# peterWon/LVI-ExC

Hardware: AMD Instinct MI355X
Metric: M residual+Jacobian evals/s per GN iter (higher is better)
Workload: dtype f64; 1 GPU; config4-full-LVI: 1000000 surfel + 200000 IMU samples (gyro+accel blocks) + 49992 ORB reprojection blocks, 25023 knots @ dt=0.02; step = residuals + analytic Jacobians + Huber + J^T J/J^T r assembly (no linear solve); n_tangent=155259, bandwidth=179, n_border=52, tracks=orb, parallelism=sequence-per-gpu x1, allreduce_transport=none (one sequence)

## Files before the change

lvi-exc_amd/csrc/lvx_api.hip:

```cpp
#include <algorithm>
#include <cmath>
#include <cstring>
#include <numeric>
#include <cstdlib>

#include "lvx_ctx.h"

namespace lvx {

#define LVX_SYNC_EVENT_FLAGS(c) hipEventDisableTiming
const SwitchName* switch_table(int* count) {
  static const SwitchName tab[] = {
    {"FORCE_LEGACY", &Switches::force_legacy, false}, {"SERIAL", &Switches::serial, false}, {"NO_GRAPH", &Switches::no_graph, false}, {"DETERMINISTIC", &Switches::deterministic, true},
    {"CLEAR_ALL", &Switches::clear_all, false}, {"SOLVER_SEQ", &Switches::solver_seq, false}, {"SOLVER_TIMING", &Switches::solver_timing, false},
    {"CHUNK_R", &Switches::chunk_r, true}, {"CHUNK_R_IMU", &Switches::chunk_r_imu, true}, {"CHUNK_R_REP", &Switches::chunk_r_rep, true}, {"CHUNK_ROWS", &Switches::chunk_rows, true}, {"REP_ROWS", &Switches::rep_rows, true}, {"REP_FUSED", &Switches::rep_fused, true}, {"SOLVER_ND", &Switches::solver_nd, false},
    {"DA_SYNC", &Switches::da_sync, false},
    {"TEST_BAD_PIVOT", &Switches::test_bad_pivot, false},
    {"TEST_COMPACT_ONE", &Switches::test_compact_one, false},
    {"TEST_LM_SCHUR_ONE", &Switches::test_lm_schur_one, false},
  };
  *count = (int)(sizeof(tab) / sizeof(tab[0]));
  return tab;
}
static void read_env_switches(lvx_ctx* c) {
  int n; const SwitchName* t = switch_table(&n);
  for (int i = 0; i < n; ++i) {
    const std::string name = std::string("LVX_") + t[i].name;
    if (const char* e = std::getenv(name.c_str())) c->sw.*(t[i].field) = (*e == 0) ? 1 : atoi(e);
  }
}

__global__ void k_checksum(const unsigned long long* p, size_t n, unsigned long long* out) {
  unsigned long long acc = 0;
  for (size_t i = (size_t)blockIdx.x * blockDim.x + threadIdx.x; i < n; i += (size_t)gridDim.x * blockDim.x) {
    unsigned long long b = p[i];
    if (b == 0x8000000000000000ull) b = 0;
    acc += b * (2ull * i + 1ull);
  }
  for (int o = 32; o > 0; o >>= 1) acc += __shfl_xor(acc, o);
  if ((threadIdx.x & 63) == 0) atomicAdd(out, acc);
}
__global__ void k_export_tail(const double* cost, const int* err, double* out) { out[0] = cost[0]; out[1] = (double)err[0]; }

}

using namespace lvx;

extern "C" {
// ... 428 lines not shown
```

lvi-exc_amd/csrc/lvx_ctx.h:

```cpp
#pragma once
#include <hip/hip_runtime.h>
#include <stdint.h>

#include <array>
#include <string>
#include <functional>
#include <vector>

#include "../../include/lvx.h"
#include "lvx_resid.h"

#define LVX_NREP 64
#define LVX_DEAD (-2147483647 - 1)
#define LVX_LM_BASE 0x40000000
#define LVX_ERR_FALLBACK 16

namespace lvx {

struct XbTab { int32_t* keys[LVX_NUM_FAM]; double* vals[LVX_NUM_FAM]; };
struct DevCommon {
  const double* state;
  int N, L;
  double t0, dt;
  uint32_t locks;
  uint32_t what;
  double imu_mto, sensor_mto;
  CamIntr cam;
  const int* ord;
  int nb, bw, nbd;
  int nbd_solve;
  int nrep;
  int hub_lo, hub_hi;
  const void* hubs;
  const So3Pre* pre;
  double* Hb;
  double* gb;
  double* Bd;
  double* C;
  double* gc;
  double* lmH; const int* lm_p0; int lm_wl, lm_ls;
  double* cost;
  int* err;
  int* fb_list; int fb_cap;
  double* residuals;
  int32_t* jcols;
  union {
    double* jvals;
    const XbTab* xb;
  };
};

struct DevBuf {
  void* p = nullptr;
  size_t bytes = 0;
};

struct Switches {
  int force_legacy = 0, serial = 0, no_graph = 0, deterministic = 0, clear_all = 0, solver_seq = 0, solver_timing = 0, chunk_r = 0, chunk_r_imu = 0, chunk_r_rep = 0, chunk_rows = 0, rep_rows = 0, da_sync = 0, rep_fused = 0, solver_nd = 0, test_bad_pivot = 0, test_compact_one = 0, test_lm_schur_one = 0;
};
struct SwitchName { const char* name; int Switches::*field; bool relayout; };
const SwitchName* switch_table(int* count);

struct Family {
  int n = 0;
  std::vector<double> t, a3, b3;
  std::vector<int32_t> id0, id1;
  double huber = 0, weight = 1;
  DevBuf d_t, d_a3, d_b3, d_id0, d_id1, d_perm;
};

}

struct lvx_ctx {
  int device = 0;
  hipStream_t stream = nullptr;
  hipStream_t own_stream = nullptr;
  hipStream_t fam_stream[4] = {nullptr, nullptr, nullptr, nullptr};
  hipEvent_t ev_fork = nullptr, ev_join[4] = {nullptr, nullptr, nullptr, nullptr}, ev_jac = nullptr;
  hipEvent_t ev_fb[2] = {nullptr, nullptr};
  std::string last_error;
  bool have_spline = false;
  double t0 = 0, dt = 1;
  int N = 0, L = 0;
  uint32_t locks = LVX_LOCK_LIDAR_TAU | LVX_LOCK_CAM_TAU;
  double imu_mto = 0.01, sensor_mto = 0.001;
  lvx::CamIntr cam{};
  lvx::Family imu, surf, rep, cs;
  lvx::Family lp; double lp_t_start = 0;
  lvx::DevBuf d_pairs_lp, d_lp_part, d_lp_out; double* h_lp = nullptr;
  bool has_prior = false;
  double prior_t = 0, prior_q[4] = {1, 0, 0, 0}, prior_w = 1;
// ... 134 lines not shown
```

lvi-exc_amd/csrc/lvx_eval.hip:

```cpp
#include <algorithm>
#include <cmath>
#include <cstring>
#include <functional>
#include <numeric>
#include <cstdlib>

#include <thread>
#include "lvx_ctx.h"

namespace lvx {

#define LVX_PW 4
struct Keys { int k0, k1, lm; };
LVX_HD bool same(const Keys& a, const Keys& b) { return a.k0 == b.k0 && a.k1 == b.k1 && a.lm == b.lm; }

struct Cal { ImuCal imu; SensorCal lidar, cam; const double* rho; };
__device__ __forceinline__ Cal load_cal(const DevCommon& cm) {
  const double* s = cm.state + 7 * (size_t)cm.N;
  Cal c;
  c.imu.tau = s[7]; c.imu.roll = s[8]; c.imu.pitch = s[9]; c.imu.ba = load_v3(s + 10); c.imu.bg = load_v3(s + 13);
  c.lidar.q = load_q(s + 16); c.lidar.p = load_v3(s + 20); c.lidar.tau = s[23];
  c.cam.q = load_q(s + 24); c.cam.p = load_v3(s + 28); c.cam.tau = s[31];
  c.rho = s + 32;
  return c;
// ... 1310 lines not shown
}

struct ImuG { enum { NR = 3, NCJ = GYRO_NC, NK = 12, NG = 3, KPK = 3, LVO = 3, GL = 32, GOFF = 5, NKL = 12, NCL = 16, NT = 1, NTP = 1, LDP = 18, PR = 96 }; };
struct ImuA { enum { NR = 3, NCJ = ACC_NC, NK = 24, NG = 5, KPK = 6, LVO = 0, GL = 16, GOFF = 0, NKL = 24, NCL = 30, NT = 2, NTP = 3, LDP = 34, PR = 48 }; };
#define IMU_NGA 8
struct ImuAccLds { double* band; double* bd; double* gg; double* gk; double* gG; int lv; };
template <class PG> __device__ __forceinline__ int imu_cls(int lc) {
  return lc < PG::NKL ? 6 * (lc / PG::KPK) + PG::LVO + lc % PG::KPK : (lc < PG::NKL + PG::NG ? -1 - (PG::GOFF + lc - PG::NKL) : (lc == PG::NKL + PG::NG ? -100 : -200));
}
template <class PG> __device__ __forceinline__ void imu_build_rtab(int* rtab, int lane, const double* sm, const ImuAccLds& A) {
  int t = 0;
#pragma unroll
  for (int ci = 0; ci < PG::NT; ++ci)
#pragma unroll
    for (int cj = ci; cj < PG::NT; ++cj, ++t)
#pragma unroll
      for (int v = 0; v < 4; ++v) {
        const int row = ci * 16 + (lane >> 4) + 4 * v, col = cj * 16 + (lane & 15);
        int ent = -1;
        if (!(ci == cj && col < row)) {
          const int ra = imu_cls<PG>(row), cb = imu_cls<PG>(col);
          if (ra >= 0) {
            if (cb >= 0) { const int d = cb - ra; if (d >= 0 && d < ACC_BW) ent = ((int)(A.band - sm) + ra * ACC_BW + d) | (2 << 16) | (cb << 18); }
            else if (cb > -100) ent = ((int)(A.bd - sm) + (-1 - cb) * A.lv + ra) | (1 << 16) | (ra << 18);
            else if (cb == -100) ent = ((int)(A.gk - sm) + ra) | (1 << 16) | (ra << 18);
          } else if (ra > -100) {
            if (cb > -100 && cb < 0) ent = (int)(A.gg - sm) + (-1 - ra) * IMU_NGA + (-1 - cb);
            else if (cb == -100) ent = (int)(A.gG - sm) + (-1 - ra);
          }
        }
        rtab[t * 4 + v] = ent;
      }
}
template <class PG> __device__ __forceinline__ void imu_assemble(double* sm, double* P, const int* rtab, bool valid, int key, int k_lo, int acc_lv, const double* r, const double (*J)[PG::NCJ], int lane, int dummy) {
  constexpr int NR = PG::NR, NT = PG::NT, LDP = PG::LDP, PR = PG::PR, GL = PG::GL;
  const unsigned long long vm = __ballot(valid);
  for (int g0 = 0; g0 < 64; g0 += GL) {
    const unsigned long long pmask = ((1ull << GL) - 1ull) << g0;
    unsigned long long rem = vm & pmask;
    if (!rem) continue;
    if (lane >= g0 && lane < g0 + GL) {
      const int li = lane - g0;
#pragma unroll
      for (int a = 0; a < NR; ++a) {
        double2* prow2 = (double2*)(P + (li * NR + a) * LDP);
        auto col = [&](int c) { return c < PG::NK + PG::NG ? (valid ? J[a][c] : 0.0) : (c == PG::NK + PG::NG ? (valid ? r[a] : 0.0) : 0.0); };
#pragma unroll
        for (int c2 = 0; c2 < 8 * NT; ++c2) prow2[c2] = make_double2(col(2 * c2), col(2 * c2 + 1));
      }
    }
    __builtin_amdgcn_fence(__ATOMIC_RELEASE, "wavefront");
    __builtin_amdgcn_wave_barrier();
    __builtin_amdgcn_fence(__ATOMIC_ACQUIRE, "wavefront");
    while (rem) {
      const int l0 = __ffsll((long long)rem) - 1;
      const int kw = __builtin_amdgcn_readfirstlane(__shfl(key, l0));
      const unsigned long long wm = __ballot(valid && key == kw) & pmask;
      rem &= ~wm;
      const int lhi = 63 - __clzll((long long)wm);
      const int wb = (kw - k_lo) * 6;
      const int r_lo = (l0 - g0) * NR, r_hi = (lhi - g0 + 1) * NR;
      const unsigned long long wsh = wm >> g0;
      const bool contig = __popcll(wm) == lhi - l0 + 1;
      d4 D[PG::NTP];
#pragma unroll
      for (int t = 0; t < PG::NTP; ++t) D[t] = d4{0.0, 0.0, 0.0, 0.0};
      const int nks = (r_hi - r_lo + 3) >> 2;
      auto trip = [&](int ks, auto UC) {
        constexpr int U = decltype(UC)::value;
        double f[U][NT];
#pragma unroll
        for (int q = 0; q < U; ++q) {
          const int rr = r_lo + 4 * (ks + q) + (lane >> 4);
          bool mine = rr < r_hi;
          if (!contig) mine = mine && ((wsh >> (rr / NR)) & 1ull);
          const double* src = P + min(rr, PR - 1) * LDP + (lane & 15);
#pragma unroll
          for (int c = 0; c < NT; ++c) { const double x = src[c * 16]; f[q][c] = mine ? x : 0.0; }
        }
#pragma unroll
        for (int q = 0; q < U; ++q) {
          int t = 0;
#pragma unroll
          for (int ci = 0; ci < NT; ++ci)
#pragma unroll
            for (int cj = ci; cj < NT; ++cj, ++t) D[t] = __builtin_amdgcn_mfma_f64_16x16x4f64(f[q][ci], f[q][cj], D[t], 0, 0, 0);
        }
      };
      int ks = 0;
      for (; ks + 6 <= nks; ks += 6) trip(ks, std::integral_constant<int, 6>{});
      for (; ks < nks; ks += 2) trip(ks, std::integral_constant<int, 2>{});
      const int wbB = wb * ACC_BW;
#pragma unroll
      for (int t = 0; t < PG::NTP; ++t)
#pragma unroll
        for (int v = 0; v < 4; ++v) {
          const int te = rtab[t * 4 + v];
          const bool ok = te >= 0 && wb + (te >> 18) < acc_lv;
          const int m = (te >> 16) & 3;
          const int idx = ok ? (te & 0xffff) + (m == 2 ? wbB : (m == 1 ? wb : 0)) : dummy + lane;
          atomicAdd(&sm[idx], ok ? D[t][v] : 0.0);
        }
    }
    __builtin_amdgcn_fence(__ATOMIC_RELEASE, "wavefront");
    __builtin_amdgcn_wave_barrier();
  }
}
struct ImuFused { int n; const double* t; const double* gyro; const double* acc; const int* perm; double w_gyro, w_acc; };
#define IMU_CR 32
#define IMU_LV ((IMU_CR + 5) * 6)
struct ImuOwn { const int* wg_c0; const int* own_k; int nch, span; };
#define LVX_LDS_BARRIER() asm volatile("s_waitcnt lgkmcnt(0)\n\ts_barrier" ::: "memory")
static size_t imu_fused_lds_bytes(int span) {
  const int pan = std::max((int)ImuG::PR * (int)ImuG::LDP, (int)ImuA::PR * (int)ImuA::LDP);
  return (size_t)(IMU_LV * ACC_BW + IMU_NGA * IMU_LV + IMU_NGA * IMU_NGA + IMU_LV + IMU_NGA + 64 + 4 * pan) * 8 + (size_t)span * sizeof(So3Pre) + (size_t)(7 * span + IMU_NGA) * 4 + 64;
}
__global__ void k_imu_rtab(int* out) {
  const int lane = threadIdx.x;
  const double* sm = (const double*)out;
  ImuAccLds A;
  A.band = (double*)sm; A.bd = A.band + IMU_LV * ACC_BW; A.gg = A.bd + IMU_NGA * IMU_LV; A.gk = A.gg + IMU_NGA * IMU_NGA; A.gG = A.gk + IMU_LV; A.lv = IMU_LV;
  int rtg[ImuG::NTP * 4], rta[ImuA::NTP * 4];
  imu_build_rtab<ImuG>(rtg, lane, sm, A);
  imu_build_rtab<ImuA>(rta, lane, sm, A);
  for (int i = 0; i < ImuG::NTP * 4; ++i) out[i * 64 + lane] = rtg[i];
  for (int i = 0; i < ImuA::NTP * 4; ++i) out[(ImuG::NTP * 4 + i) * 64 + lane] = rta[i];
}
template <bool EXP = false>
__global__ __launch_bounds__(256, 1) void k_imu_own(ImuFused fam, DevCommon cm, const int* __restrict__ chunk_off, ImuOwn ow, long long row0_g, long long row0_a, int det, const int* __restrict__ rtab_g) {
  constexpr int PAN = (ImuG::PR * ImuG::LDP > ImuA::PR * ImuA::LDP) ? ImuG::PR * ImuG::LDP : ImuA::PR * ImuA::LDP;
  constexpr int ACC_LV = IMU_LV, CR = IMU_CR, HB = ACC_BW / 2;
  extern __shared__ __attribute__((aligned(16))) double smo[];
  double* sm = smo;
  ImuAccLds A;
  A.band = sm; A.bd = A.band + ACC_LV * ACC_BW; A.gg = A.bd + IMU_NGA * ACC_LV; A.gk = A.gg + IMU_NGA * IMU_NGA; A.gG = A.gk + ACC_LV; A.lv = ACC_LV;
  double* panels = A.gG + IMU_NGA + 64;
  So3Pre* pre_all = (So3Pre*)(panels + 4 * PAN);
  int* kpos_all = (int*)(pre_all + ow.span);
  int* kown_all = kpos_all + 6 * ow.span;
  int* gpos = kown_all + ow.span;
  const int tid = threadIdx.x, lane = tid & 63, wv = tid >> 6;
  const int wg = blockIdx.x;
  const int c0 = ow.wg_c0[wg], c1 = ow.wg_c0[wg + 1];
  if (c0 >= c1) return;
  const int nwv = det ? 1 : 4;
  const bool want_ne = (cm.what & LVX_EVAL_NORMAL_EQ) != 0;
  constexpr int NACC = ACC_LV * ACC_BW + IMU_NGA * ACC_LV + IMU_NGA * IMU_NGA + ACC_LV + IMU_NGA;
  for (int e = tid; e < NACC; e += 256) sm[e] = 0.0;
  int* urng = gpos + IMU_NGA;
  if (tid < IMU_NGA) gpos[tid] = cm.ord[6 * cm.N + tid];
  if (tid == 0) { urng[0] = 1 << 30; urng[1] = -1; }
  const int k_base = chunk_off[ow.nch + 1 + c0] - 1;
  for (int e = tid; e < 6 * ow.span; e += 256) { const int kn = k_base + e / 6; kpos_all[e] = (kn >= 0 && kn < cm.N) ? cm.ord[6 * kn + e % 6] : LVX_DEAD; }
  for (int e = tid; e < ow.span; e += 256) {
    const int kn = k_base + e;
    kown_all[e] = (ow.own_k && kn >= 0 && kn < cm.N) ? ow.own_k[kn] : -1;
    if (kn >= 0 && kn + 1 < cm.N) pre_all[e] = cm.pre[kn];
    else { pre_all[e].Om = mk(0, 0, 0); pre_all[e].on = 0.0; pre_all[e].Jri = m3_identity(); pre_all[e].c3 = 1.0 / 12.0; pre_all[e].ok = 1; }
  }
  const SplineRef sp{cm.t0, cm.dt, cm.N, cm.state, cm.state + 3 * (size_t)cm.N};
  const Cal cal = load_cal(cm);
  if (fabs(cal.imu.tau) >= cm.dt && tid == 0) atomicOr(cm.err, LVX_ERR_FALLBACK);
  double* P = panels + wv * PAN;
  const int rep = wg % cm.nrep;
  int rtg[ImuG::NTP * 4], rta[ImuA::NTP * 4];
#pragma unroll
  for (int i = 0; i < ImuG::NTP * 4; ++i) rtg[i] = rtab_g[i * 64 + lane];
#pragma unroll
  for (int i = 0; i < ImuA::NTP * 4; ++i) rta[i] = rtab_g[(ImuG::NTP * 4 + i) * 64 + lane];
  double mycost = 0.0;
  const int ld = cm.bw + 1;
#ifdef LVX_KTIME_IMU
  long long kt_[12] = {0, 0, 0, 0, 0, 0, 0, 0, 0, 0, 0, 0}; long long kt0_ = __builtin_amdgcn_s_memtime(); const long long kts_ = kt0_;
#define IKT(i) { const long long n_ = __builtin_amdgcn_s_memtime(); kt_[i] += n_ - kt0_; kt0_ = n_; }
#else
#define IKT(i)
#endif
  for (int c = c0; c < c1; ++c) {
    const int m0 = chunk_off[c], m1 = chunk_off[c + 1];
    const int k_lo = chunk_off[ow.nch + 1 + c] - 1;
    const int woff = k_lo - k_base;
    const So3Pre* pre_tab = pre_all + woff;
    const int* kpos = kpos_all + 6 * woff;
    if (c == c0) __syncthreads(); else LVX_LDS_BARRIER();
    IKT(0)
    for (int base = wv < nwv ? m0 + wv * 64 : m1; base < m1; base += nwv * 64) {
      const int si = base + lane;
      const bool in = si < m1;
      int key = -1;
      bool valid = false;
      So3Eval e;
      KnotRef k;
      if (in) {
        int status = RES_OK;
        if (!knot_lookup(sp.t0, sp.dt, sp.n, fam.t[si], fam.t[si] + cal.imu.tau, &k)) status = RES_RANGE;
        else {
          key = k.i0;
          const So3Pre* pre = (k.i0 >= k_lo && k.i0 + 2 < k_lo + CR + 4) ? pre_tab + (k.i0 - k_lo) : nullptr;
          if (!pre) status = RES_OUTSIDE;
          else {
            quat cq[4]; load_so3_cp(sp, k.i0, cq);
            const int bad = so3_eval_pre<true, true>(cq, pre, k.u, sp.dt, &e);
            if (bad) status = (bad & 1) ? RES_NONUNIT : RES_OUTSIDE;
          }
        }
        valid = status == RES_OK;
        if (valid && (key < k_lo || key - k_lo > CR + 1)) { valid = false; fallback_row(cm, LVX_FAM_GYRO, si); }
        else if (!valid && status == RES_OUTSIDE) fallback_row(cm, LVX_FAM_GYRO, si);
        else if (!valid) atomicOr(cm.err, status);
      }
      IKT(1)
      {
        double r[3], J[3][GYRO_NC];
        if (valid) {
          const v3 wm = load_v3(fam.gyro + 3 * (size_t)si);
          const v3 pred = e.w_body + cal.imu.bg;
          const double w = fam.w_gyro;
          r[0] = w * (wm.x - pred.x); r[1] = w * (wm.y - pred.y); r[2] = w * (wm.z - pred.z);
#pragma unroll
          for (int kk = 0; kk < 4; ++kk)
#pragma unroll
            for (int a = 0; a < 3; ++a)
#pragma unroll
              for (int b = 0; b < 3; ++b) J[a][3 * kk + b] = -w * e.dw[kk].a[3 * a + b];
#pragma unroll
          for (int a = 0; a < 3; ++a)
#pragma unroll
            for (int b = 0; b < 3; ++b) J[a][12 + b] = (a == b) ? -w : 0.0;
          mycost += 0.5 * (r[0] * r[0] + r[1] * r[1] + r[2] * r[2]);
          if (cm.residuals) { const long long orow = row0_g + (long long)fam.perm[si] * 3; cm.residuals[orow] = r[0]; cm.residuals[orow + 1] = r[1]; cm.residuals[orow + 2] = r[2]; }
          if constexpr (EXP) put_record<3, GYRO_NC>(cm, LVX_FAM_GYRO, fam.perm[si], key, -1, -1, [&](int a, int c) { return J[a][c]; });
        }
        if constexpr (EXP) { if (in && !valid) { put_skipped(cm, LVX_FAM_GYRO, fam.perm[si]); put_skipped(cm, LVX_FAM_ACCEL, fam.perm[si]); } }
        if (want_ne) imu_assemble<ImuG>(sm, P, rtg, valid, key, k_lo, ACC_LV, r, J, lane, NACC);
        IKT(2)
      }
      {
        double r[3], J[3][ACC_NC];
        if (valid) {
          R3Basis b; r3_basis(k.u, sp.dt, &b);
          v3 acc = mk(0, 0, 0);
#pragma unroll
          for (int j = 0; j < 4; ++j) acc = acc + b.Ba[j] * load_v3(sp.r3 + 3 * (k.i0 + j));
          const v3 am = load_v3(fam.acc + 3 * (size_t)si);
          const double w = fam.w_acc;
          const double G = -9.79;
          const double cr = cos(cal.imu.roll), sr = sin(cal.imu.roll), cp = cos(cal.imu.pitch), sp_ = sin(cal.imu.pitch);
          const v3 g = mk(-sp_ * cr * G, sr * G, -cr * cp * G);
          const v3 y = acc + g;
          const v3 yb = qrot_inv(e.q, y);
          const v3 pred = yb + cal.imu.ba;
          r[0] = w * (am.x - pred.x); r[1] = w * (am.y - pred.y); r[2] = w * (am.z - pred.z);
          const m3 Rt = transpose(rotmat(e.q));
          const m3 S = skew(yb);
#pragma unroll
          for (int kk = 0; kk < 4; ++kk) {
            const m3 Mx = S * e.dxi[kk];
#pragma unroll
            for (int a = 0; a < 3; ++a)
#pragma unroll
              for (int bb = 0; bb < 3; ++bb) { J[a][6 * kk + bb] = -w * b.Ba[kk] * Rt.a[3 * a + bb]; J[a][6 * kk + 3 + bb] = -w * Mx.a[3 * a + bb]; }
          }
          const v3 dg_dr = Rt * mk(sp_ * sr * G, cr * G, sr * cp * G);
          const v3 dg_dp = Rt * mk(-cp * cr * G, 0.0, cr * sp_ * G);
#pragma unroll
          for (int a = 0; a < 3; ++a) {
            J[a][24] = -w * comp(dg_dr, a); J[a][25] = -w * comp(dg_dp, a);
#pragma unroll
            for (int bb = 0; bb < 3; ++bb) J[a][26 + bb] = (a == bb) ? -w : 0.0;
          }
          mycost += 0.5 * (r[0] * r[0] + r[1] * r[1] + r[2] * r[2]);
          if (cm.residuals) { const long long orow = row0_a + (long long)fam.perm[si] * 3; cm.residuals[orow] = r[0]; cm.residuals[orow + 1] = r[1]; cm.residuals[orow + 2] = r[2]; }
          if constexpr (EXP) put_record<3, ACC_NC>(cm, LVX_FAM_ACCEL, fam.perm[si], key, -1, -1, [&](int a, int c) { return J[a][c]; });
        }
        if (want_ne) imu_assemble<ImuA>(sm, P, rta, valid, key, k_lo, ACC_LV, r, J, lane, NACC);
        IKT(3)
      }
    }
    if (!want_ne) continue;
    int bt = tid; asm volatile("" : "+v"(bt));
    const bool more = c + 1 < c1;
    const int nfl = more ? min(ACC_LV, max(0, 6 * (chunk_off[ow.nch + 1 + c + 1] - 1 - k_lo))) : ACC_LV;
    const int* kown = kown_all + woff;
    const bool un_ = bt < nfl && kpos[bt] != LVX_DEAD && kown[bt / 6] != wg;
    { const unsigned long long ub = __ballot(un_);
      if (ub && lane == 0) { atomicMin(&urng[0], wv * 64 + __ffsll((long long)ub) - 1); atomicMax(&urng[1], wv * 64 + 63 - __clzll((long long)ub)); } }
    const int any_unowned = __syncthreads_or(un_);
    IKT(4)
    if (any_unowned) {
      const int r0 = urng[0], r1 = urng[1] + 1;
      for (int e = r0 * ACC_BW + bt; e < r1 * ACC_BW; e += 256) {
        const int la = e / ACC_BW, lb = la + e % ACC_BW;
        const int pa = kpos[la], o = kown[la / 6];
        if (o == wg || pa == LVX_DEAD || lb >= ACC_LV) continue;
        const double v = A.band[e];
        if (v == 0.0) continue;
        if (o >= 0) { atomicOr(cm.err, LVX_ERR_FALLBACK); continue; }
        const int pb = kpos[lb];
        if (pb != LVX_DEAD) add_H(cm, pa, pb, v, rep);
      }
      for (int gi = 0; gi < IMU_NGA; ++gi)
        for (int la = r0 + bt; la < r1; la += 256) {
          const int pg = gpos[gi], pa = kpos[la], o = kown[la / 6];
          if (pg == LVX_DEAD || pa == LVX_DEAD || (o == wg && pg < 0)) continue;
          const double v = A.bd[gi * ACC_LV + la];
          if (v == 0.0) continue;
          if (o >= 0) atomicOr(cm.err, LVX_ERR_FALLBACK); else add_H(cm, pg, pa, v, rep);
        }
      if (bt < nfl && kpos[bt] != LVX_DEAD && kown[bt / 6] != wg) {
        const double v = A.gk[bt];
        if (v != 0.0) { if (kown[bt / 6] >= 0) atomicOr(cm.err, LVX_ERR_FALLBACK); else add_g(cm, kpos[bt], v, rep); }
      }
      LVX_LDS_BARRIER();
      if (tid == 0) { urng[0] = 1 << 30; urng[1] = -1; }
    }
    IKT(6)
    {
      constexpr int NQB = (ACC_LV * HB + 255) / 256, NQD = (IMU_NGA * ACC_LV + 255) / 256;
      double2* band2 = (double2*)A.band;
      double2 vb[NQB]; int pb_[NQB], ob_[NQB];
#pragma unroll
      for (int q = 0; q < NQB; ++q) {
        const int e2 = bt + 256 * q;
        const bool inr = e2 < ACC_LV * HB;
        const int la = inr ? e2 / HB : 0;
        vb[q] = inr ? band2[e2] : make_double2(0.0, 0.0);
        pb_[q] = kpos[la]; ob_[q] = kown[la / 6];
        if (inr && more) band2[e2] = make_double2(0.0, 0.0);
      }
      double vd[NQD], vg = 0.0; int pd_[NQD], od_[NQD], pg_ = LVX_DEAD, og_ = -1;
#pragma unroll
      for (int q = 0; q < NQD; ++q) {
        const int e = bt + 256 * q;
        const bool inr = e < IMU_NGA * ACC_LV;
        const int la = inr ? e % ACC_LV : 0;
        vd[q] = inr ? A.bd[e] : 0.0;
        pd_[q] = kpos[la]; od_[q] = kown[la / 6];
        if (inr && more) A.bd[e] = 0.0;
      }
      if (bt < ACC_LV) { vg = A.gk[bt]; pg_ = kpos[bt]; og_ = kown[bt / 6]; if (more) A.gk[bt] = 0.0; }
      int gp_[NQD];
#pragma unroll
      for (int q = 0; q < NQD; ++q) { const int e = bt + 256 * q; gp_[q] = gpos[e < IMU_NGA * ACC_LV ? e / ACC_LV : 0]; }
      LVX_LDS_BARRIER();
      IKT(7)
#pragma unroll
      for (int q = 0; q < NQB; ++q) {
        const int e2 = bt + 256 * q;
        const int la = e2 / HB, d = 2 * (e2 % HB);
// ... 297 lines not shown
}

static void stable_perm_by_key(const std::vector<int>& key, std::vector<int>& perm) {
  const size_t n = key.size();
  perm.resize(n);
  if (n == 0) return;
  int lo = key[0], hi = key[0];
  for (size_t i = 1; i < n; ++i) { lo = std::min(lo, key[i]); hi = std::max(hi, key[i]); }
  if ((long long)hi - lo > (long long)(4 * n + 1024)) {
    std::iota(perm.begin(), perm.end(), 0);
    std::stable_sort(perm.begin(), perm.end(), [&](int a, int b) { return key[a] < key[b]; });
    return;
  }
  std::vector<int> cnt((size_t)(hi - lo) + 2, 0);
  for (size_t i = 0; i < n; ++i) cnt[(size_t)(key[i] - lo) + 1]++;
  for (size_t k = 1; k < cnt.size(); ++k) cnt[k] += cnt[k - 1];
  for (size_t i = 0; i < n; ++i) perm[(size_t)cnt[(size_t)(key[i] - lo)]++] = (int)i;
}
int ensure_layout(lvx_ctx* ctx) {
  if (!ctx->layout_dirty) return LVX_OK;
  if (!ctx->have_spline) return fail(ctx, LVX_E_STATE, "lvx_set_spline has not been called");
  const int N = ctx->N, L = ctx->L;
  const uint32_t locks = ctx->locks;
  int rc;
  {
    const long long npl = (long long)ctx->planes.size() / 3;
    for (int i = 0; i < ctx->surf.n; ++i) if (ctx->surf.id0[i] < 0 || ctx->surf.id0[i] >= npl) return fail(ctx, LVX_E_ARG, "surfel plane id out of range for the current plane table");
    for (int i = 0; i < ctx->cs.n; ++i) {
      if (ctx->cs.id1[i] < 0 || ctx->cs.id1[i] >= npl) return fail(ctx, LVX_E_ARG, "cam-surfel plane id out of range for the current plane table");
      if (ctx->cs.id0[i] < 0 || ctx->cs.id0[i] >= L) return fail(ctx, LVX_E_ARG, "cam-surfel landmark id out of range for the current landmark table");
    }
  }
  const SplineRef sp{ctx->t0, ctx->dt, N, nullptr, nullptr};
  {
    Family& f = ctx->imu;
    std::vector<int> key(f.n), perm(f.n);
    par_for((size_t)f.n, [&](size_t a, size_t b) { for (size_t i = a; i < b; ++i) key[i] = host_i0(ctx, f.t[i]); });
    stable_perm_by_key(key, perm);
    { std::vector<int> sk(f.n); for (int i = 0; i < f.n; ++i) sk[i] = key[perm[i]];
      if ((rc = upload_chunks(ctx, LVX_FAM_GYRO, sk, pick_chunk_batches(16, 64, ctx->sw.chunk_r_imu, (double)f.n / std::max(1, N - 3), 4 * (int)GyroAcc::LB)))) return rc;
      const int ncu = ctx->n_cu;
      const int cr = IMU_CR;
      std::vector<int> off, k0, wg_c0;
      int G = std::max(1, std::min(ncu, (f.n + 255) / 256)), span = 0;
      for (;; G *= 2) {
        off.clear(); k0.clear(); wg_c0.clear(); span = cr + 5;
        int r = 0;
        for (int g = 0; g < G; ++g) {
          wg_c0.push_back((int)k0.size());
          int r1 = g + 1 == G ? f.n : (int)((long long)f.n * (g + 1) / G);
          while (r1 < f.n && r1 > 0 && sk[r1] == sk[r1 - 1]) ++r1;
          r1 = std::max(r1, r);
          const size_t first = k0.size();
          for (int i = r; i < r1;) {
            const int kf = std::max(0, sk[i]);
            int e = std::min(r1, i + 256);
            while (e > i + 1 && sk[e - 1] >= kf + cr) --e;
            off.push_back(i); k0.push_back(kf);
            i = e;
          }
          if (k0.size() > first) span = std::max(span, k0.back() - k0[first] + cr + 5);
          r = r1;
        }
        wg_c0.push_back((int)k0.size());
        if (imu_fused_lds_bytes(span) <= 160 * 1024 || G >= std::max(1, f.n)) break;
      }
      ctx->imu_wg = G; ctx->imu_nch = (int)k0.size(); ctx->imu_span = span; ctx->imu_h_k0 = k0; ctx->imu_h_wg_c0 = wg_c0;
      off.push_back(f.n);
      off.insert(off.end(), k0.begin(), k0.end());
      if ((rc = upload_tmp(ctx, ctx->d_imu_chunk, off.data(), off.size() * 4))) return rc;
      if ((rc = upload_tmp(ctx, ctx->d_imu_wg, wg_c0.data(), wg_c0.size() * 4))) return rc;
    }
    auto ts = gather(f.t, perm, 1); auto g = gather(f.a3, perm, 3); auto a = gather(f.b3, perm, 3);
    if ((rc = upload_tmp(ctx, f.d_t, ts.data(), ts.size() * 8))) return rc;
    if ((rc = upload_tmp(ctx, f.d_a3, g.data(), g.size() * 8))) return rc;
    if ((rc = upload_tmp(ctx, f.d_b3, a.data(), a.size() * 8))) return rc;
    if ((rc = upload_tmp(ctx, f.d_perm, perm.data(), perm.size() * 4))) return rc;
  }
  {
    Family& f = ctx->surf;
    std::vector<int> key(f.n), perm(f.n);
    par_for((size_t)f.n, [&](size_t a, size_t b) { for (size_t i = a; i < b; ++i) key[i] = host_i0(ctx, f.t[i]); });
    stable_perm_by_key(key, perm);
    { std::vector<int> sk(f.n); for (int i = 0; i < f.n; ++i) sk[i] = key[perm[i]]; if (ctx->sw.chunk_r) rc = upload_chunks(ctx, LVX_FAM_SURFEL, sk, pick_chunk(ctx, 8, 16, ctx->sw.chunk_r, 2, 2.2));
      else rc = upload_chunks_rows(ctx, LVX_FAM_SURFEL, sk, 16, ctx->sw.chunk_rows > 0 ? ctx->sw.chunk_rows : 512);
      if (rc) return rc; }
    auto ts = gather(f.t, perm, 1); auto pt = gather(f.a3, perm, 3); auto pl = gather(f.id0, perm, 1);
    if ((rc = upload_tmp(ctx, f.d_t, ts.data(), ts.size() * 8))) return rc;
    if ((rc = upload_tmp(ctx, f.d_a3, pt.data(), pt.size() * 8))) return rc;
    if ((rc = upload_tmp(ctx, f.d_id0, pl.data(), pl.size() * 4))) return rc;
    if ((rc = upload_tmp(ctx, f.d_perm, perm.data(), perm.size() * 4))) return rc;
    std::vector<double> rowpl((size_t)f.n * 3, 0.0);
    const long long npl = (long long)ctx->planes.size() / 3;
    par_for((size_t)f.n, [&](size_t a, size_t b) { for (size_t i = a; i < b; ++i) if (pl[i] >= 0 && pl[i] < npl) for (int c = 0; c < 3; ++c) rowpl[3 * i + c] = ctx->planes[3 * (size_t)pl[i] + c]; });
    if ((rc = upload_tmp(ctx, f.d_b3, rowpl.data(), rowpl.size() * 8))) return rc;
  }
  {
    Family& f = ctx->rep;
    const double row_delta = ctx->cam.rows > 0 ? ctx->cam.readout / (double)ctx->cam.rows : 0.0;
    std::vector<int> k1(f.n), k0(f.n), perm(f.n);
    for (int i = 0; i < f.n; ++i) {
      const int l = f.id0[i];
      k1[i] = host_i0(ctx, f.t[i] + f.a3[2 * (size_t)i + 1] * row_delta);
      k0[i] = (l >= 0 && l < L) ? host_i0(ctx, ctx->lm_t0[l] + ctx->lm_uv[2 * (size_t)l + 1] * row_delta) : -1;
// ... 200 lines not shown
    std::vector<int> goff;
    int spread = 0;
    for (size_t i = 0; i < order.size(); ++i) {
      if (goff.empty() || (int)i - goff.back() >= 32 || lm_p0[order[i]] - lm_p0[order[goff.back()]] > 24) goff.push_back((int)i);
      spread = std::max(spread, lm_p0[order[i]] - lm_p0[order[goff.back()]]);
    }
    ctx->lm_ngrp = (int)goff.size(); ctx->lm_gspread = spread;
    goff.push_back((int)order.size());
    goff.insert(goff.end(), order.begin(), order.end());
    if ((rc = upload_tmp(ctx, ctx->d_lm_grp, goff.data(), goff.size() * 4))) return rc;
  }
  if ((rc = upload_tmp(ctx, ctx->d_lm_p0, lm_p0.data(), lm_p0.size() * 4))) return rc;
  if ((rc = dev_alloc(ctx, ctx->d_lmH, (size_t)std::max(L, 1) * ctx->lm_ls * 8 + 16))) return rc;
  ctx->bw = std::min(std::max(bw, 0), std::max(ctx->nb - 1, 0));
  ctx->clear_npre = std::min(bw_near, ctx->bw) + 1;
  {
    int reach = 5;
    for (int i = 0; i < ctx->rep.n; ++i) reach = std::max(reach, rep_kmax[i] - rep_kmin[i] + 2);
    int lo = 1 << 30, hi = -1;
    if (nh > 0) span_pos(std::max(0, h0 - reach), std::min(N - 1, h0 + nh + reach), lo, hi);
    ctx->hub_near_lo = hi >= lo ? lo : 0; ctx->hub_near_hi = hi >= lo ? hi + 1 : 0;
  }
  if ((rc = upload_tmp(ctx, ctx->d_colfull, colfull.data(), colfull.size()))) return rc;
  {
    ctx->h_colhi.assign((size_t)std::max(ctx->nb, 0), 0);
    int run = -1;
    for (int j = 0; j < ctx->nb; ++j) { run = std::max(run, top[j]); ctx->h_colhi[j] = std::max(run, j); }
    ctx->h_colfull.assign(colfull.begin(), colfull.begin() + std::max(ctx->nb, 0));
    ctx->bw_near = std::min(bw_near, ctx->bw);
    ++ctx->layout_epoch;
  }
  {
    std::vector<int> own((size_t)std::max(ctx->nb, 1), -1), own_k((size_t)std::max(N, 1), -1);
    const int G = ctx->imu_wg, cr = IMU_CR;
    const std::vector<int>& k0 = ctx->imu_h_k0; const std::vector<int>& wc = ctx->imu_h_wg_c0;
    ctx->imu_owned_cols = 0;
    if (ctx->nb > 0 && !(locks & LVX_LOCK_R3) && ctx->imu.n > 0 && ctx->dt > ctx->imu_mto) {
      int prev = -1;
      for (int g = 0; g < G; ++g) {
        if (wc[g] >= wc[g + 1]) continue;
        int nxt = -1; for (int h = g + 1; h < G && nxt < 0; ++h) if (wc[h] < wc[h + 1]) nxt = h;
        const int lo = prev < 0 ? 0 : k0[wc[g]] + 4, hi = nxt < 0 ? N - 1 : k0[wc[nxt]] - 2;
        for (int c = wc[g]; c < wc[g + 1]; ++c)
          for (int k = std::max(lo, k0[c] - 1); k <= std::min(hi, k0[c] - 1 + cr + 4); ++k) {
            if (k < 0 || k + 4 >= N) continue;
            const int p0 = ctx->ord[6 * k];
            if (p0 < 0 || p0 >= LVX_LM_BASE) continue;
            bool contig = true;
            for (int e = 0; e < 30 && contig; ++e) contig = ctx->ord[6 * k + e] == p0 + e;
            if (!contig) continue;
            for (int d = 0; d < 6; ++d) { if (own[p0 + d] < 0) ctx->imu_owned_cols++; own[p0 + d] = g; }
            own_k[k] = g;
          }
        prev = g;
      }
    }
    ctx->imu_own_k_off = own.size();
    own.insert(own.end(), own_k.begin(), own_k.end());
    if ((rc = upload_tmp(ctx, ctx->d_imu_own, own.data(), own.size() * 4))) return rc;
  }
  ctx->bd_row_live.assign((size_t)ctx->nbd_ext, 0);
  for (int b = 0; b < 6 * nh; ++b) ctx->bd_row_live[b] = 1;
  for (int c = 0; c < 22; ++c) if (ctx->ord[6 * N + c] != LVX_DEAD) ctx->bd_row_live[6 * nh + c] = 1;
  for (int p = 0; p < 6; ++p) { ctx->bd_row_live[ctx->nbd + p] = ctx->surf.n > 0; ctx->bd_row_live[ctx->nbd + 6 + p] = ctx->cs.n > 0; }
  ctx->nrep = LVX_NREP;
  for (auto& v : ctx->det_col) v.clear();
  if (ctx->sw.deterministic) {
    int need = std::max(LVX_NREP, (ctx->rep.n + 63) / 64);
    for (size_t q = 0; q + 1 < ctx->det_cross_col.size(); ++q) need = std::max(need, ctx->det_cross_col[q + 1] - ctx->det_cross_col[q]);
    for (int slot : {LVX_FAM_GYRO, LVX_FAM_SURFEL, LVX_FAM_CAMSURF, LVX_FAM_REPROJ, LVX_FAM_PRIOR}) {
      const int nch = ctx->n_chunk[slot];
      if (nch <= 0 || (int)ctx->h_chunk_k0[slot].size() != nch) continue;
      const int span = ctx->chunk_r[slot] + 5;
      std::vector<std::vector<uint8_t>> occ; std::vector<std::vector<int>> members;
      for (int c = 0; c < nch; ++c) {
        if (ctx->h_chunk_rows[slot][c] <= 0) continue;
        const int lo = std::max(0, ctx->h_chunk_k0[slot][c] - 1), hi = std::min(N, ctx->h_chunk_k0[slot][c] - 1 + span);
        size_t col = 0;
        for (; col < occ.size(); ++col) { bool hit = false; for (int k = lo; k < hi && !hit; ++k) hit = occ[col][k] != 0; if (!hit) break; }
        if (col == occ.size()) { occ.emplace_back((size_t)N, (uint8_t)0); members.emplace_back(); }
        for (int k = lo; k < hi; ++k) occ[col][k] = 1;
        members[col].push_back(c);
      }
      std::vector<int> list; ctx->det_col[slot].push_back(0);
      for (auto& m : members) { list.insert(list.end(), m.begin(), m.end()); ctx->det_col[slot].push_back((int)list.size()); }
      if (list.empty()) { ctx->det_col[slot].clear(); continue; }
      if ((rc = upload_tmp(ctx, ctx->d_det_list[slot], list.data(), list.size() * 4))) return rc;
      need = std::max(need, nch);
// ... 544 lines not shown
```

Measured before the change: 2762 Mevals/s.

## Give IMU workgroups halo samples so boundary knots stay workgroup-owned

Reworks the IMU chunk partition so each workgroup also evaluates a small halo of samples just before its primary range. The halo rows contribute only to that workgroup's local normal-equation accumulator and are not counted for cost or residual output. Boundary knots can then be owned exclusively by one workgroup, which shrinks the slow global atomic add_H/add_g flush of unowned entries. Per-wave sample slices are now precomputed on the host and aligned to knot boundaries instead of fixed 64-sample strides. The cost is redundant residual and Jacobian evaluation on the halo rows, plus a more complex host-side layout pass.

```diff
diff --git a/lvi-exc_amd/csrc/lvx_api.hip b/lvi-exc_amd/csrc/lvx_api.hip
--- a/lvi-exc_amd/csrc/lvx_api.hip
+++ b/lvi-exc_amd/csrc/lvx_api.hip
@@ -14,6 +14,7 @@
     {"FORCE_LEGACY", &Switches::force_legacy, false}, {"SERIAL", &Switches::serial, false}, {"NO_GRAPH", &Switches::no_graph, false}, {"DETERMINISTIC", &Switches::deterministic, true},
     {"CLEAR_ALL", &Switches::clear_all, false}, {"SOLVER_SEQ", &Switches::solver_seq, false}, {"SOLVER_TIMING", &Switches::solver_timing, false},
     {"CHUNK_R", &Switches::chunk_r, true}, {"CHUNK_R_IMU", &Switches::chunk_r_imu, true}, {"CHUNK_R_REP", &Switches::chunk_r_rep, true}, {"CHUNK_ROWS", &Switches::chunk_rows, true}, {"REP_ROWS", &Switches::rep_rows, true}, {"REP_FUSED", &Switches::rep_fused, true}, {"SOLVER_ND", &Switches::solver_nd, false},
+    {"IMU_FIXED_SLICES", &Switches::imu_fixed_slices, true},
     {"DA_SYNC", &Switches::da_sync, false},
     {"TEST_BAD_PIVOT", &Switches::test_bad_pivot, false},
     {"TEST_COMPACT_ONE", &Switches::test_compact_one, false},
diff --git a/lvi-exc_amd/csrc/lvx_ctx.h b/lvi-exc_amd/csrc/lvx_ctx.h
--- a/lvi-exc_amd/csrc/lvx_ctx.h
+++ b/lvi-exc_amd/csrc/lvx_ctx.h
@@ -56,7 +56,7 @@
 };
 
 struct Switches {
-  int force_legacy = 0, serial = 0, no_graph = 0, deterministic = 0, clear_all = 0, solver_seq = 0, solver_timing = 0, chunk_r = 0, chunk_r_imu = 0, chunk_r_rep = 0, chunk_rows = 0, rep_rows = 0, da_sync = 0, rep_fused = 0, solver_nd = 0, test_bad_pivot = 0, test_compact_one = 0, test_lm_schur_one = 0;
+  int force_legacy = 0, serial = 0, no_graph = 0, deterministic = 0, clear_all = 0, solver_seq = 0, solver_timing = 0, chunk_r = 0, chunk_r_imu = 0, chunk_r_rep = 0, chunk_rows = 0, rep_rows = 0, da_sync = 0, rep_fused = 0, solver_nd = 0, test_bad_pivot = 0, test_compact_one = 0, test_lm_schur_one = 0, imu_fixed_slices = 0;
 };
 struct SwitchName { const char* name; int Switches::*field; bool relayout; };
 const SwitchName* switch_table(int* count);
diff --git a/lvi-exc_amd/csrc/lvx_eval.hip b/lvi-exc_amd/csrc/lvx_eval.hip
--- a/lvi-exc_amd/csrc/lvx_eval.hip
+++ b/lvi-exc_amd/csrc/lvx_eval.hip
@@ -1366,7 +1366,7 @@
         rtab[t * 4 + v] = ent;
       }
 }
-template <class PG> __device__ __forceinline__ void imu_assemble(double* sm, double* P, const int* rtab, bool valid, int key, int k_lo, int acc_lv, const double* r, const double (*J)[PG::NCJ], int lane, int dummy) {
+template <class PG, bool HALO> __device__ __forceinline__ void imu_assemble(double* sm, double* P, const int* rtab, bool valid, int key, int k_lo, int acc_lv, const double* r, const double (*J)[PG::NCJ], int lane, int dummy, int nhalo) {
   constexpr int NR = PG::NR, NT = PG::NT, LDP = PG::LDP, PR = PG::PR, GL = PG::GL;
   const unsigned long long vm = __ballot(valid);
   for (int g0 = 0; g0 < 64; g0 += GL) {
@@ -1425,13 +1425,14 @@
       for (; ks + 6 <= nks; ks += 6) trip(ks, std::integral_constant<int, 6>{});
       for (; ks < nks; ks += 2) trip(ks, std::integral_constant<int, 2>{});
       const int wbB = wb * ACC_BW;
+      const int mlo = l0 < nhalo ? 1 : 0;
 #pragma unroll
       for (int t = 0; t < PG::NTP; ++t)
 #pragma unroll
         for (int v = 0; v < 4; ++v) {
           const int te = rtab[t * 4 + v];
-          const bool ok = te >= 0 && wb + (te >> 18) < acc_lv;
           const int m = (te >> 16) & 3;
+          const bool ok = te >= 0 && (!HALO || m >= mlo) && wb + (te >> 18) < acc_lv;
           const int idx = ok ? (te & 0xffff) + (m == 2 ? wbB : (m == 1 ? wb : 0)) : dummy + lane;
           atomicAdd(&sm[idx], ok ? D[t][v] : 0.0);
         }
@@ -1479,6 +1480,8 @@
   if (c0 >= c1) return;
   const int nwv = det ? 1 : 4;
   const bool want_ne = (cm.what & LVX_EVAL_NORMAL_EQ) != 0;
+  const int prim0 = ow.wg_c0[gridDim.x + 1 + wg];
+  const bool use_halo = ow.own_k != nullptr && want_ne;
   constexpr int NACC = ACC_LV * ACC_BW + IMU_NGA * ACC_LV + IMU_NGA * IMU_NGA + ACC_LV + IMU_NGA;
   for (int e = tid; e < NACC; e += 256) sm[e] = 0.0;
   int* urng = gpos + IMU_NGA;
@@ -1511,16 +1514,20 @@
 #define IKT(i)
 #endif
   for (int c = c0; c < c1; ++c) {
-    const int m0 = chunk_off[c], m1 = chunk_off[c + 1];
+    const int m0 = chunk_off[c], m1 = chunk_off[2 * ow.nch + 1 + c];
     const int k_lo = chunk_off[ow.nch + 1 + c] - 1;
     const int woff = k_lo - k_base;
     const So3Pre* pre_tab = pre_all + woff;
     const int* kpos = kpos_all + 6 * woff;
     if (c == c0) __syncthreads(); else LVX_LDS_BARRIER();
     IKT(0)
-    for (int base = wv < nwv ? m0 + wv * 64 : m1; base < m1; base += nwv * 64) {
+    const int* so = chunk_off + 3 * ow.nch + 1 + 5 * c;
+    const int wvu = __builtin_amdgcn_readfirstlane(wv);
+    const int b1 = nwv == 1 ? m1 : so[wvu + 1];
+    for (int base = nwv == 1 ? (wvu == 0 ? m0 : m1) : so[wvu]; base < b1; base += 64) {
       const int si = base + lane;
-      const bool in = si < m1;
+      const bool hal = si < prim0;
+      const bool in = si < b1 && (use_halo || !hal);
       int key = -1;
       bool valid = false;
       So3Eval e;
@@ -1539,10 +1546,13 @@
           }
         }
         valid = status == RES_OK;
-        if (valid && (key < k_lo || key - k_lo > CR + 1)) { valid = false; fallback_row(cm, LVX_FAM_GYRO, si); }
-        else if (!valid && status == RES_OUTSIDE) fallback_row(cm, LVX_FAM_GYRO, si);
-        else if (!valid) atomicOr(cm.err, status);
-      }
+        if (valid && (key < k_lo || key - k_lo > CR + 1)) { valid = false; status = RES_OUTSIDE; }
+        if (!valid && !hal) {
+          if (status == RES_OUTSIDE) fallback_row(cm, LVX_FAM_GYRO, si);
+          else atomicOr(cm.err, status);
+        }
+      }
+      const bool mine = valid && !hal;
       IKT(1)
       {
         double r[3], J[3][GYRO_NC];
@@ -1561,12 +1571,14 @@
           for (int a = 0; a < 3; ++a)
 #pragma unroll
             for (int b = 0; b < 3; ++b) J[a][12 + b] = (a == b) ? -w : 0.0;
-          mycost += 0.5 * (r[0] * r[0] + r[1] * r[1] + r[2] * r[2]);
-          if (cm.residuals) { const long long orow = row0_g + (long long)fam.perm[si] * 3; cm.residuals[orow] = r[0]; cm.residuals[orow + 1] = r[1]; cm.residuals[orow + 2] = r[2]; }
-          if constexpr (EXP) put_record<3, GYRO_NC>(cm, LVX_FAM_GYRO, fam.perm[si], key, -1, -1, [&](int a, int c) { return J[a][c]; });
-        }
-        if constexpr (EXP) { if (in && !valid) { put_skipped(cm, LVX_FAM_GYRO, fam.perm[si]); put_skipped(cm, LVX_FAM_ACCEL, fam.perm[si]); } }
-        if (want_ne) imu_assemble<ImuG>(sm, P, rtg, valid, key, k_lo, ACC_LV, r, J, lane, NACC);
+          if (mine) {
+            mycost += 0.5 * (r[0] * r[0] + r[1] * r[1] + r[2] * r[2]);
+            if (cm.residuals) { const long long orow = row0_g + (long long)fam.perm[si] * 3; cm.residuals[orow] = r[0]; cm.residuals[orow + 1] = r[1]; cm.residuals[orow + 2] = r[2]; }
+            if constexpr (EXP) put_record<3, GYRO_NC>(cm, LVX_FAM_GYRO, fam.perm[si], key, -1, -1, [&](int a, int c) { return J[a][c]; });
+          }
+        }
+        if constexpr (EXP) { if (in && !valid && !hal) { put_skipped(cm, LVX_FAM_GYRO, fam.perm[si]); put_skipped(cm, LVX_FAM_ACCEL, fam.perm[si]); } }
+        if (want_ne) { if (base < prim0) imu_assemble<ImuG, true>(sm, P, rtg, valid, key, k_lo, ACC_LV, r, J, lane, NACC, prim0 - base); else imu_assemble<ImuG, false>(sm, P, rtg, valid, key, k_lo, ACC_LV, r, J, lane, NACC, 0); }
         IKT(2)
       }
       {
@@ -1603,11 +1615,13 @@
 #pragma unroll
             for (int bb = 0; bb < 3; ++bb) J[a][26 + bb] = (a == bb) ? -w : 0.0;
           }
-          mycost += 0.5 * (r[0] * r[0] + r[1] * r[1] + r[2] * r[2]);
-          if (cm.residuals) { const long long orow = row0_a + (long long)fam.perm[si] * 3; cm.residuals[orow] = r[0]; cm.residuals[orow + 1] = r[1]; cm.residuals[orow + 2] = r[2]; }
-          if constexpr (EXP) put_record<3, ACC_NC>(cm, LVX_FAM_ACCEL, fam.perm[si], key, -1, -1, [&](int a, int c) { return J[a][c]; });
-        }
-        if (want_ne) imu_assemble<ImuA>(sm, P, rta, valid, key, k_lo, ACC_LV, r, J, lane, NACC);
+          if (mine) {
+            mycost += 0.5 * (r[0] * r[0] + r[1] * r[1] + r[2] * r[2]);
+            if (cm.residuals) { const long long orow = row0_a + (long long)fam.perm[si] * 3; cm.residuals[orow] = r[0]; cm.residuals[orow + 1] = r[1]; cm.residuals[orow + 2] = r[2]; }
+            if constexpr (EXP) put_record<3, ACC_NC>(cm, LVX_FAM_ACCEL, fam.perm[si], key, -1, -1, [&](int a, int c) { return J[a][c]; });
+          }
+        }
+        if (want_ne) { if (base < prim0) imu_assemble<ImuA, true>(sm, P, rta, valid, key, k_lo, ACC_LV, r, J, lane, NACC, prim0 - base); else imu_assemble<ImuA, false>(sm, P, rta, valid, key, k_lo, ACC_LV, r, J, lane, NACC, 0); }
         IKT(3)
       }
     }
@@ -1616,7 +1630,7 @@
     const bool more = c + 1 < c1;
     const int nfl = more ? min(ACC_LV, max(0, 6 * (chunk_off[ow.nch + 1 + c + 1] - 1 - k_lo))) : ACC_LV;
     const int* kown = kown_all + woff;
-    const bool un_ = bt < nfl && kpos[bt] != LVX_DEAD && kown[bt / 6] != wg;
+    const bool un_ = bt < nfl && kpos[bt] != LVX_DEAD && kown[bt / 6] < 0;
     { const unsigned long long ub = __ballot(un_);
       if (ub && lane == 0) { atomicMin(&urng[0], wv * 64 + __ffsll((long long)ub) - 1); atomicMax(&urng[1], wv * 64 + 63 - __clzll((long long)ub)); } }
     const int any_unowned = __syncthreads_or(un_);
@@ -1626,29 +1640,27 @@
       for (int e = r0 * ACC_BW + bt; e < r1 * ACC_BW; e += 256) {
         const int la = e / ACC_BW, lb = la + e % ACC_BW;
         const int pa = kpos[la], o = kown[la / 6];
-        if (o == wg || pa == LVX_DEAD || lb >= ACC_LV) continue;
+        if (o >= 0 || pa == LVX_DEAD || lb >= ACC_LV) continue;
         const double v = A.band[e];
         if (v == 0.0) continue;
-        if (o >= 0) { atomicOr(cm.err, LVX_ERR_FALLBACK); continue; }
         const int pb = kpos[lb];
         if (pb != LVX_DEAD) add_H(cm, pa, pb, v, rep);
       }
       for (int gi = 0; gi < IMU_NGA; ++gi)
         for (int la = r0 + bt; la < r1; la += 256) {
           const int pg = gpos[gi], pa = kpos[la], o = kown[la / 6];
-          if (pg == LVX_DEAD || pa == LVX_DEAD || (o == wg && pg < 0)) continue;
+          if (pg == LVX_DEAD || pa == LVX_DEAD || (o >= 0 && (o != wg || pg < 0))) continue;
           const double v = A.bd[gi * ACC_LV + la];
-          if (v == 0.0) continue;
-          if (o >= 0) atomicOr(cm.err, LVX_ERR_FALLBACK); else add_H(cm, pg, pa, v, rep);
-        }
-      if (bt < nfl && kpos[bt] != LVX_DEAD && kown[bt / 6] != wg) {
+          if (v != 0.0) add_H(cm, pg, pa, v, rep);
+        }
+      if (bt < nfl && kpos[bt] != LVX_DEAD && kown[bt / 6] < 0) {
         const double v = A.gk[bt];
-        if (v != 0.0) { if (kown[bt / 6] >= 0) atomicOr(cm.err, LVX_ERR_FALLBACK); else add_g(cm, kpos[bt], v, rep); }
+        if (v != 0.0) add_g(cm, kpos[bt], v, rep);
       }
       LVX_LDS_BARRIER();
       if (tid == 0) { urng[0] = 1 << 30; urng[1] = -1; }
-    }
-    IKT(6)
+      IKT(6)
+    }
     {
       constexpr int NQB = (ACC_LV * HB + 255) / 256, NQD = (IMU_NGA * ACC_LV + 255) / 256;
       double2* band2 = (double2*)A.band;
@@ -2012,6 +2024,7 @@
     }
   }
   const SplineRef sp{ctx->t0, ctx->dt, N, nullptr, nullptr};
+  std::vector<int> imu_sk;
   {
     Family& f = ctx->imu;
     std::vector<int> key(f.n), perm(f.n);
@@ -2019,37 +2032,7 @@
     stable_perm_by_key(key, perm);
     { std::vector<int> sk(f.n); for (int i = 0; i < f.n; ++i) sk[i] = key[perm[i]];
       if ((rc = upload_chunks(ctx, LVX_FAM_GYRO, sk, pick_chunk_batches(16, 64, ctx->sw.chunk_r_imu, (double)f.n / std::max(1, N - 3), 4 * (int)GyroAcc::LB)))) return rc;
-      const int ncu = ctx->n_cu;
-      const int cr = IMU_CR;
-      std::vector<int> off, k0, wg_c0;
-      int G = std::max(1, std::min(ncu, (f.n + 255) / 256)), span = 0;
-      for (;; G *= 2) {
-        off.clear(); k0.clear(); wg_c0.clear(); span = cr + 5;
-        int r = 0;
-        for (int g = 0; g < G; ++g) {
-          wg_c0.push_back((int)k0.size());
-          int r1 = g + 1 == G ? f.n : (int)((long long)f.n * (g + 1) / G);
-          while (r1 < f.n && r1 > 0 && sk[r1] == sk[r1 - 1]) ++r1;
-          r1 = std::max(r1, r);
-          const size_t first = k0.size();
-          for (int i = r; i < r1;) {
-            const int kf = std::max(0, sk[i]);
-            int e = std::min(r1, i + 256);
-            while (e > i + 1 && sk[e - 1] >= kf + cr) --e;
-            off.push_back(i); k0.push_back(kf);
-            i = e;
-          }
-          if (k0.size() > first) span = std::max(span, k0.back() - k0[first] + cr + 5);
-          r = r1;
-        }
-        wg_c0.push_back((int)k0.size());
-        if (imu_fused_lds_bytes(span) <= 160 * 1024 || G >= std::max(1, f.n)) break;
-      }
-      ctx->imu_wg = G; ctx->imu_nch = (int)k0.size(); ctx->imu_span = span; ctx->imu_h_k0 = k0; ctx->imu_h_wg_c0 = wg_c0;
-      off.push_back(f.n);
-      off.insert(off.end(), k0.begin(), k0.end());
-      if ((rc = upload_tmp(ctx, ctx->d_imu_chunk, off.data(), off.size() * 4))) return rc;
-      if ((rc = upload_tmp(ctx, ctx->d_imu_wg, wg_c0.data(), wg_c0.size() * 4))) return rc;
+      imu_sk.swap(sk);
     }
     auto ts = gather(f.t, perm, 1); auto g = gather(f.a3, perm, 3); auto a = gather(f.b3, perm, 3);
     if ((rc = upload_tmp(ctx, f.d_t, ts.data(), ts.size() * 8))) return rc;
@@ -2316,28 +2299,106 @@
   }
   {
     std::vector<int> own((size_t)std::max(ctx->nb, 1), -1), own_k((size_t)std::max(N, 1), -1);
-    const int G = ctx->imu_wg, cr = IMU_CR;
-    const std::vector<int>& k0 = ctx->imu_h_k0; const std::vector<int>& wc = ctx->imu_h_wg_c0;
+    const Family& f = ctx->imu;
+    const std::vector<int>& sk = imu_sk;
+    const int cr = IMU_CR;
+    const bool can_own = ctx->nb > 0 && !(locks & LVX_LOCK_R3) && f.n > 0 && ctx->dt > ctx->imu_mto;
+    std::vector<char> free_k((size_t)std::max(N, 1), 0);
+    if (can_own)
+      for (int k = 0; k + 4 < N; ++k) {
+        const int p0 = ctx->ord[6 * k];
+        if (p0 < 0 || p0 >= LVX_LM_BASE) continue;
+        bool contig = true;
+        for (int e = 0; e < 30 && contig; ++e) contig = ctx->ord[6 * k + e] == p0 + e;
+        free_k[k] = contig;
+      }
+    std::vector<int> off, k0, end, sl, wc, rb, halo, ws;
+    auto slices = [&](int i, int e) {
+      const size_t s0 = sl.size();
+      for (int w = 0; w <= 4; ++w) sl.push_back(std::min(e, i + 64 * w));
+      if (ctx->sw.imu_fixed_slices) return;
+      ws.clear();
+      for (int s = i; s < e; ++s) if (s == i || sk[s] != sk[s - 1]) ws.push_back(s);
+      ws.push_back(e);
+      const int nw = (int)ws.size() - 1, q = nw / 4, x = nw % 4;
+      for (int mask = 0; mask < 16; ++mask) {
+        if (__builtin_popcount(mask) != x) continue;
+        int cut[5] = {i, 0, 0, 0, 0}, p = 0;
+        bool ok = true;
+        for (int w = 0; w < 4; ++w) { p += q + ((mask >> w) & 1); cut[w + 1] = ws[p]; ok = ok && cut[w + 1] - cut[w] <= 64; }
+        if (!ok) continue;
+        std::copy(cut, cut + 5, sl.begin() + s0);
+        return;
+      }
+    };
+    std::vector<char> shared;
+    int G = std::max(1, std::min(ctx->n_cu, (f.n + 255) / 256)), span = 0;
+    for (;; G *= 2) {
+      rb.assign(1, 0);
+      for (int g = 0; g < G; ++g) {
+        int r1 = g + 1 == G ? f.n : (int)((long long)f.n * (g + 1) / G);
+        while (r1 < f.n && r1 > 0 && sk[r1] == sk[r1 - 1]) ++r1;
+        rb.push_back(std::max(r1, rb.back()));
+      }
+      halo.assign(G, 0); shared.assign((size_t)std::max(N, 1), 0);
+      for (int g = 1; g < G; ++g) halo[g] = can_own && rb[g] > 0 && rb[g] < rb[g + 1] && sk[rb[g]] >= 0;
+      for (bool changed = can_own; changed;) {
+        changed = false;
+        for (int g = 1; g < G; ++g) {
+          if (!halo[g]) continue;
+          const int P0 = sk[rb[g]];
+          bool ok = true;
+          for (int k = std::max(0, P0 - 3); k <= std::min(N - 1, P0 + 2) && ok; ++k) ok = free_k[k] && !shared[k];
+          if (ok) continue;
+          halo[g] = 0; changed = true;
+          for (int k = P0; k <= std::min(N - 1, P0 + 2); ++k) shared[k] = 1;
+        }
+      }
+      off.clear(); k0.clear(); end.clear(); sl.clear(); wc.clear(); span = cr + 5;
+      for (int g = 0; g < G; ++g) {
+        wc.push_back((int)k0.size());
+        const int r0 = halo[g] ? (int)(std::lower_bound(sk.begin(), sk.begin() + rb[g], std::max(0, sk[rb[g]] - 3)) - sk.begin()) : rb[g], r1 = rb[g + 1];
+        const size_t first = k0.size();
+        for (int i = r0; i < r1;) {
+          const int kf = std::max(0, sk[i]);
+          int e = std::min(r1, i + 256);
+          while (e > i + 1 && sk[e - 1] >= kf + cr) --e;
+          off.push_back(i); k0.push_back(kf); end.push_back(e);
+          slices(i, e);
+          i = e;
+        }
+        if (k0.size() > first) span = std::max(span, k0.back() - k0[first] + cr + 5);
+      }
+      wc.push_back((int)k0.size());
+      if (imu_fused_lds_bytes(span) <= 160 * 1024 || G >= std::max(1, f.n)) break;
+    }
+    ctx->imu_wg = G; ctx->imu_nch = (int)k0.size(); ctx->imu_span = span; ctx->imu_h_k0 = k0; ctx->imu_h_wg_c0 = wc;
     ctx->imu_owned_cols = 0;
-    if (ctx->nb > 0 && !(locks & LVX_LOCK_R3) && ctx->imu.n > 0 && ctx->dt > ctx->imu_mto) {
+    if (can_own) {
       int prev = -1;
       for (int g = 0; g < G; ++g) {
-        if (wc[g] >= wc[g + 1]) continue;
-        int nxt = -1; for (int h = g + 1; h < G && nxt < 0; ++h) if (wc[h] < wc[h + 1]) nxt = h;
-        const int lo = prev < 0 ? 0 : k0[wc[g]] + 4, hi = nxt < 0 ? N - 1 : k0[wc[nxt]] - 2;
+        if (rb[g] >= rb[g + 1]) continue;
+        int nxt = -1; for (int h = g + 1; h < G && nxt < 0; ++h) if (rb[h] < rb[h + 1]) nxt = h;
+        const int lo = prev < 0 ? 0 : sk[rb[g]], hi = nxt < 0 ? N - 1 : sk[rb[nxt]] - 1;
         for (int c = wc[g]; c < wc[g + 1]; ++c)
           for (int k = std::max(lo, k0[c] - 1); k <= std::min(hi, k0[c] - 1 + cr + 4); ++k) {
-            if (k < 0 || k + 4 >= N) continue;
+            if (k < 0 || k >= N || !free_k[k] || shared[k]) continue;
             const int p0 = ctx->ord[6 * k];
-            if (p0 < 0 || p0 >= LVX_LM_BASE) continue;
-            bool contig = true;
-            for (int e = 0; e < 30 && contig; ++e) contig = ctx->ord[6 * k + e] == p0 + e;
-            if (!contig) continue;
             for (int d = 0; d < 6; ++d) { if (own[p0 + d] < 0) ctx->imu_owned_cols++; own[p0 + d] = g; }
             own_k[k] = g;
           }
         prev = g;
       }
+    }
+    {
+      std::vector<int> wgtab(wc);
+      wgtab.insert(wgtab.end(), rb.begin(), rb.begin() + G);
+      off.push_back(f.n);
+      off.insert(off.end(), k0.begin(), k0.end());
+      off.insert(off.end(), end.begin(), end.end());
+      off.insert(off.end(), sl.begin(), sl.end());
+      if ((rc = upload_tmp(ctx, ctx->d_imu_chunk, off.data(), off.size() * 4))) return rc;
+      if ((rc = upload_tmp(ctx, ctx->d_imu_wg, wgtab.data(), wgtab.size() * 4))) return rc;
     }
     ctx->imu_own_k_off = own.size();
     own.insert(own.end(), own_k.begin(), own_k.end());
```

Measured after the change: 2806 Mevals/s (median of 6 runs). 1.02x the previous value.
